# Sanoojan/REFace

Measured on AMD Instinct MI355X. Metric: 512x512 50-step DDIM images/sec, higher is better.
Workload: dtype bf16; 1 GPU; BASELINE configs[1]: 512x512, 50 DDIM steps, CFG scale 3.5, batch 8 per GPU, bf16 UNet + fp32 VAE decode (bf16x3 MFMA operands), seeded random-init REFace weights; id=c1:512x512:S50:B8:bf16, batch_per_gpu=8, global_batch=8, ddim_steps=50, latent=64, parallelism=dp1 (pairs sharded, no collective in the step loop)

## Files before the change

reface_amd/csrc/gemm.hip:

```cpp
#include <cstdlib>
#include <type_traits>

#include "common.h"
#include "gemm_plan.h"


namespace rf {
typedef float f32x2_t __attribute__((ext_vector_type(2)));


typedef __attribute__((ext_vector_type(2))) __bf16 bf16x2v_t;
__device__ __forceinline__ u32x4_t fp8x8_to_bf16x8(const u32x2_t& r, float scale) {
    u32x4_t o;
    o[0] = __builtin_bit_cast(uint32_t, __builtin_amdgcn_cvt_scalef32_pk_bf16_fp8(r[0], scale, false));
    o[1] = __builtin_bit_cast(uint32_t, __builtin_amdgcn_cvt_scalef32_pk_bf16_fp8(r[0], scale, true));
    o[2] = __builtin_bit_cast(uint32_t, __builtin_amdgcn_cvt_scalef32_pk_bf16_fp8(r[1], scale, false));
    o[3] = __builtin_bit_cast(uint32_t, __builtin_amdgcn_cvt_scalef32_pk_bf16_fp8(r[1], scale, true));
    return o;
}

template <typename T> struct MmaFrag;
template <> struct MmaFrag<bf16_t> {
    __device__ static __forceinline__ void mma(f32x16_t& acc, const u32x4_t& a, const u32x4_t& b) {
        acc = __builtin_amdgcn_mfma_f32_32x32x16_bf16(__builtin_bit_cast(bf16x8_t, a), __builtin_bit_cast(bf16x8_t, b), acc, 0, 0, 0);
// ... 27 lines not shown

__device__ __forceinline__ int lds_off(int row, int slot) { return row * 128 + ((slot ^ ((row >> 1) & 7)) << 4); }

template <bool W8> __device__ __forceinline__ int w_stage(int t, int buf) { return W8 ? ((t >> 1) & 1) : buf; }
template <bool W8> __device__ __forceinline__ int w_soff(int t) { return (W8 ? (t >> 1) : t) * 128; }

template <typename TO> __device__ __forceinline__ void store_out(TO* p, float v);
template <> __device__ __forceinline__ void store_out<float>(float* p, float v) { *p = v; }
template <> __device__ __forceinline__ void store_out<bf16_t>(bf16_t* p, float v) { *p = f2bf(v); }
template <> __device__ __forceinline__ void store_out<f16_t>(f16_t* p, float v) { *p = (f16_t)v; }
template <typename TO> __device__ __forceinline__ float load_out(const TO* p);
template <> __device__ __forceinline__ float load_out<float>(const float* p) { return *p; }
template <> __device__ __forceinline__ float load_out<bf16_t>(const bf16_t* p) { return bf2f(*p); }
template <> __device__ __forceinline__ float load_out<f16_t>(const f16_t* p) { return (float)*p; }
template <typename X> struct is16 { static constexpr bool value = std::is_same<X, bf16_t>::value || std::is_same<X, f16_t>::value; };

template <typename T, typename TO, int WM, int WN, int TM, int TN, bool CONV, bool GLDS, int NST, int EPI = 0, bool W8 = false, int LNF = 0, bool HX = false>
__global__ __launch_bounds__(WM* WN * 64) void conv_gemm_kernel(const GemmParams p) {
    static_assert(LNF == 0 || (EPI == 1 && !CONV && !W8 && sizeof(T) == 2 && sizeof(TO) == 2), "LayerNorm folding: bf16 linear layers on the direct epilogue");
    static_assert(!HX || (CONV && GLDS && NST == 2 && sizeof(T) == 2 && !W8), "row-extended A tiles: bf16 3x3 convolutions on the two-stage direct-to-LDS loop");
    static_assert(EPI == 0 || GLDS, "the direct epilogue is built on the direct-to-LDS main loop");
    static_assert(!W8 || (GLDS && std::is_same<T, bf16_t>::value), "fp8 weights: bf16 activations on the direct-to-LDS main loop");
    constexpr bool A8 = std::is_same<T, fp8_t>::value;
    static_assert(!A8 || (GLDS && !W8 && NST == 2), "fp8 activations: direct-to-LDS main loop, two stages");
    constexpr int NT = WM * WN * 64;
    constexpr int BM = 32 * TM * WM;
    constexpr int BN = 32 * TN * WN;
    constexpr int VEC = elem<T>::VEC;
    constexpr int BK = 8 * VEC;
    constexpr int RPP = NT / 8;
// ... 25 lines not shown
        const int h = min(p.pm, p.tiles_m - sr * p.pm);
        const int pw = h * p.pn;
        const int pc = rem / pw, r2 = rem - pc * pw;
        const int c = r2 / h;
        tile_m = sr * p.pm + (r2 - c * h);
        tile_n = pc * p.pn + c;
    }
    const int m0 = tile_m * BM, n0 = tile_n * BN;

    const long long zb = blockIdx.y;
    const T* src0 = (const T*)p.src0 + zb * p.sA;
    const T* src1 = (const T*)p.src1;
    const T* Wp = W8 ? (const T*)((const char*)p.W + zb * p.sW) : (const T*)p.W + zb * p.sW;
    if (!W8 && p.w_ps) Wp += (long long)(m0 / p.rows_per_sample) * p.w_ps;
    const int hw_in = p.Hin * p.Win;
    const int uph = (CONV && p.ups == 2) ? (m0 / hw_in) & 3 : 0;
    if (!W8 && uph) Wp += (long long)uph * p.N * p.ldw;
    const bool up2 = CONV && p.ups == 2;
    const int pad_t = up2 ? 1 - (uph >> 1) : p.pad_t, pad_l = up2 ? 1 - (uph & 1) : p.pad_l;
    auto out_row = [&](int row) -> int {
        if (!up2) return row;
        const int s4 = m0 / (4 * hw_in), r = row - (s4 * 4 + uph) * hw_in;
        const int i = r / p.Win, j = r - i * p.Win;
        return (s4 * p.Hout + 2 * i + (uph >> 1)) * p.Wout + 2 * j + (uph & 1);
    };

    float colc = 0.f;
    if constexpr (EPI == 1) {
        if (tid < BN && n0 + tid < p.N && p.splitk == 1) {
            if (p.bias) colc = p.bias[n0 + tid];
            if (p.rowvec) colc += p.rowvec[(long long)(m0 / p.rows_per_sample) * p.ldv + n0 + tid];
        }
    }
    float colu = 0.f;
    if constexpr (LNF == 2) {
        if (tid < BN && n0 + tid < p.N) colu = p.ln_u[n0 + tid];
    }
    const int r0 = tid >> 3;
    const int slot = GLDS ? ((tid & 7) ^ ((r0 >> 1) & 7)) : (tid & 7);

// ... 159 lines not shown
#pragma unroll
            for (int j = 0; j < BV; ++j)
                __builtin_amdgcn_raw_ptr_buffer_load_lds(rsB, (__attribute__((address_space(3))) void*)(b0 + j * (RPP * 128)), 16, offs[AV + j], so0, 0, 0);
        }
#pragma unroll
        for (int i = 0; i < AV; ++i) {
            const int m = m0 + r0 + i * RPP;
            if constexpr (HX) {
                const int j = r0 + i * RPP, we = p.Wout + 2;
                const int ir = j / we, xc = j - ir * we;
                const int R = m0 / p.Wout + ir;
                const int b = R / p.Hout, oy = R - b * p.Hout;
                rowd[i] = (ir < BM / p.Wout && R * p.Wout < p.M) ? ((unsigned)b << 20 | (unsigned)oy << 10 | (unsigned)xc) : ~0u;
            } else if (CONV) {
                const int hw = p.Hout * p.Wout;
                const int b = m / hw;
                int rem = m - b * hw, wd = p.Wout;
                if (up2) { rem -= uph * hw_in; wd = p.Win; }
                const int oy = rem / wd, ox = rem - oy * wd;
                rowd[i] = m < p.M ? ((unsigned)b << 20 | (unsigned)oy << 10 | (unsigned)ox) : ~0u;
            } else {
                offs[i] = m < p.M ? m * p.ld0 * (int)sizeof(T) + lane_k : OOB;
            }
        }
        auto set_grp = [&](int dy, int ld) {
#pragma unroll
            for (int i = 0; i < AV; ++i) {
                const unsigned d = rowd[i];
                const int iy = (int)((d >> 10) & 1023u) + dy - 1, ix = (int)(d & 1023u) - 1;
                const bool ok = d != ~0u && (unsigned)iy < (unsigned)p.Hin && (unsigned)ix < (unsigned)p.Win;
                offs[i] = ok ? (((int)(d >> 20) * p.Hin + iy) * p.Win + ix) * ld * (int)sizeof(T) + lane_k : OOB;
            }
        };
// ... 618 lines not shown
                        gx[16 + k] = q;
                    }
                }
                if (gn_on) {
                    halfwave_reduce_scatter32(gx, lrow);
                    gcs[((lrow >> 4) * WM + wm) * BN + (wn * TN + j) * 32 + lhalf * 16 + (lrow & 15)] = gx[0];
                }
            }
            if (gn_on) {
                lds_barrier();
                if (tid < 64) {
                    const int c = tid >> 5, g = tid & 31;
                    if (p.gn_part[c]) {
                        const int cpg = p.gn_cpg[c], base = p.gn_coff[c] + n0;
                        const int lo = max(0, g * cpg - base), hi = min(min(BN, p.N - n0), (g + 1) * cpg - base);
                        double sa = 0.0, sq = 0.0;
                        for (int k = lo; k < hi; ++k)
#pragma unroll
                            for (int r = 0; r < WM; ++r) { sa += (double)gcs[r * BN + k]; sq += (double)gcs[(WM + r) * BN + k]; }
                        const int b = m0 / p.gn_rows, mt = (m0 - b * p.gn_rows) / BM;
                        double* o = p.gn_part[c] + (((long long)b * p.gn_nch[c] + p.gn_slot[c] + mt * p.tiles_n + tile_n) * 32 + g) * 2;
                        o[0] = sa;
                        o[1] = sq;
                    }
                }
            }
            if constexpr (ln_p) {
                const int part = (n0 + wn * TN * 32) / (TN * 32);
#pragma unroll
                for (int i = 0; i < TM; ++i) {
                    float sm = 0.f;
#pragma unroll
                    for (int j = 0; j < TN; ++j)
#pragma unroll
                        for (int e = 0; e < 16; ++e) sm += acc[i][j][e];
                    {
                        const auto sw = __builtin_amdgcn_permlane32_swap(as_u32(sm), as_u32(sm), false, false);
                        sm = as_f32(sw[0]) + as_f32(sw[1]);
// ... 123 lines not shown
        float cadd[4] = {0.f, 0.f, 0.f, 0.f};
        const bool rv_uniform = p.rowvec && (p.rows_per_sample % ER == 0);
        if (t_on) {
            const float* rvu = rv_uniform ? p.rowvec + (long long)(mch / p.rows_per_sample) * p.ldv : nullptr;
            if (full) {
                if (p.bias) { const f32x4_t b4 = *(const f32x4_t*)(p.bias + col); cadd[0] = b4[0]; cadd[1] = b4[1]; cadd[2] = b4[2]; cadd[3] = b4[3]; }
                if (rvu) { const f32x4_t r4 = *(const f32x4_t*)(rvu + col); cadd[0] += r4[0]; cadd[1] += r4[1]; cadd[2] += r4[2]; cadd[3] += r4[3]; }
            } else {
#pragma unroll
                for (int e = 0; e < 4; ++e)
                    if (col + e < p.N) { if (p.bias) cadd[e] = p.bias[col + e]; if (rvu) cadd[e] += rvu[col + e]; }
            }
        }
        typedef typename std::conditional<sizeof(TO) == 2, u32x2_t, f32x4_t>::type resv_t;
        int orow_cur = 0, oj = 0, ostep = 0, ostep_j = 0;
        if (up2) {
            const int r = (mch + er) % hw_in, ostep_i = EROWS / p.Win;
            orow_cur = out_row(mch + er);
            oj = r % p.Win;
            ostep_j = EROWS - ostep_i * p.Win;
            ostep = 2 * ostep_i * p.Wout + 2 * ostep_j;
        }
#pragma unroll 1
        for (int k0 = 0; k0 < PASSES; k0 += U) {
            resv_t rq[U];
            bool ok[U];
#pragma unroll
            for (int u = 0; u < U; ++u) {
                const int rl = er + (k0 + u) * EROWS, row = mch + rl;
                ok[u] = t_on && (k0 + u) < PASSES && rl < ER && row < p.M;
                if (ok[u] && resp && full) rq[u] = *(const resv_t*)(resp + (long long)row * p.ldr + col);
            }
#pragma unroll
            for (int u = 0; u < U; ++u) {
                const int orow_u = orow_cur;
                if (up2) {
                    orow_cur += ostep; oj += ostep_j;
                    if (oj >= p.Win) { oj -= p.Win; orow_cur += p.Wout; }
                }
                if (!ok[u]) continue;
                const int rl = er + (k0 + u) * EROWS, row = mch + rl;
                const f32x4_t a4 = *(const f32x4_t*)(stage + rl * BN + cl);
                float v[4] = {a4[0] * p.alpha + cadd[0], a4[1] * p.alpha + cadd[1], a4[2] * p.alpha + cadd[2], a4[3] * p.alpha + cadd[3]};
                if (p.rowvec && !rv_uniform) {
                    const float* rv = p.rowvec + (long long)(row / p.rows_per_sample) * p.ldv;
#pragma unroll
                    for (int e = 0; e < 4; ++e) if (col + e < p.N) v[e] += rv[col + e];
                }
                if (p.act != RF_ACT_NONE) {
#pragma unroll
                    for (int e = 0; e < 4; ++e) {
                        float y = v[e];
                        if (p.act == RF_ACT_SILU) y = silu_exact(y);
                        else if (p.act == RF_ACT_QUICK_GELU) y = quick_gelu(y);
                        else if (p.act == RF_ACT_GELU) y = gelu_erf(y);
                        else if (p.act == RF_ACT_RELU) y = fmaxf(y, 0.0f);
// ... 59 lines not shown
            for (int e = 0; e < 4; ++e) {
                cs[er * BN + cs_ * 4 + e] = gsum[e];
                cs[(EROWS + er) * BN + cs_ * 4 + e] = gsq[e];
            }
        }
        lds_barrier();
        if (tid < 64) {
            const int c = tid >> 5, g = tid & 31;
            if (p.gn_part[c]) {
                const int cpg = p.gn_cpg[c], base = p.gn_coff[c] + n0;
                const int lo = max(0, g * cpg - base), hi = min(min(BN, p.N - n0), (g + 1) * cpg - base);
                double sa = 0.0, sq = 0.0;
                for (int k = lo; k < hi; ++k)
#pragma unroll
                    for (int r = 0; r < EROWS; ++r) { sa += (double)cs[r * BN + k]; sq += (double)cs[(EROWS + r) * BN + k]; }
                const int b = m0 / p.gn_rows, mt = (m0 - b * p.gn_rows) / BM;
                double* o = p.gn_part[c] + (((long long)b * p.gn_nch[c] + p.gn_slot[c] + mt * p.tiles_n + tile_n) * 32 + g) * 2;
                o[0] = sa;
                o[1] = sq;
            }
        }
    }
}

template <typename TO, int SKR>
__global__ __launch_bounds__(256) void splitk_reduce_kernel(const GemmParams p) {
    const int tid = threadIdx.x;
    const int cl = (tid & 63) * 4, rp = tid >> 6;
    const int n0 = blockIdx.x * SK_COLS, m0 = blockIdx.y * SKR;
    const int col = n0 + cl;
    const bool vec = (p.N & 3) == 0 && p.vec_ok;
// ... 135 lines not shown
    for (int z = 1; z < p.splitk; ++z) {
        src += zstride;
        f32x4_t b[4];
#pragma unroll
        for (int q = 0; q < 4; ++q) b[q] = src[q * 64];
#pragma unroll
        for (int q = 0; q < 4; ++q) a[q] += b[q];
    }
    const bool live = row < p.M && col < p.N;
    const bool gn_on = p.gn_rows > 0;
    constexpr int OV = sizeof(TO) == 2 ? 2 : 4, E = 16 / OV;
    float y[16];
#pragma unroll
    for (int e = 0; e < 16; ++e) y[e] = 0.f;
    if (live) {
        TO* const dst = (TO*)p.out + (long long)row * p.ldo + col;
        const TO* const resp = p.residual ? (const TO*)p.residual + (long long)row * p.ldr + col : nullptr;
        const float* const rv = p.rowvec ? p.rowvec + (long long)(row / p.rows_per_sample) * p.ldv + col : nullptr;
        u32x4_t rq[OV];
        if (resp) {
#pragma unroll
            for (int h = 0; h < OV; ++h) rq[h] = ((const u32x4_t*)resp)[h];
        }
#pragma unroll
        for (int q = 0; q < 4; ++q) {
            f32x4_t c = {0.f, 0.f, 0.f, 0.f};
            if (p.bias) c = ((const f32x4_t*)(p.bias + col))[q];
            if (rv) c += ((const f32x4_t*)rv)[q];
#pragma unroll
            for (int e = 0; e < 4; ++e) y[4 * q + e] = a[q][e] * p.alpha + c[e];
        }
// ... 15 lines not shown
    if (gn_on) {
        __shared__ float gcs[2][32 * TN];
        float gx[32];
#pragma unroll
        for (int k = 0; k < 16; ++k) { gx[k] = y[k]; gx[16 + k] = y[k] * y[k]; }
        halfwave_reduce_scatter32(gx, lrow);
        gcs[lrow >> 4][j * 32 + lhalf * 16 + (lrow & 15)] = gx[0];
        __syncthreads();
        if (tid < 64) {
            const int c = tid >> 5, g = tid & 31;
            if (p.gn_part[c] && row0 < p.M && coln0 < p.N) {
                const int cpg = p.gn_cpg[c], base = p.gn_coff[c] + coln0;
                const int lo = max(0, g * cpg - base), hi = min(min(32 * TN, p.N - coln0), (g + 1) * cpg - base);
                double sa = 0.0, sq = 0.0;
                for (int k = lo; k < hi; ++k) { sa += (double)gcs[0][k]; sq += (double)gcs[1][k]; }
                const int b = row0 / p.gn_rows, mt = (row0 - b * p.gn_rows) / 32;
                const int nstripe = (p.N + 32 * TN - 1) / (32 * TN);
                double* o = p.gn_part[c] + (((long long)b * p.gn_nch[c] + p.gn_slot[c] + mt * nstripe + coln0 / (32 * TN)) * 32 + g) * 2;
                o[0] = sa;
                o[1] = sq;
            }
        }
    }
}

#ifdef RF_KERNEL_ONLY
}
#else
template <typename T, typename TO, int TI, bool W8>
static int launch_cfg(const GemmPart& g, const GemmParams& p, bool conv, int batch, hipStream_t st) {
    constexpr GemmTile TILE = GEMM_TILE[TI];
// ... 195 lines not shown
```

reface_amd/csrc/gemm_plan.h:

```cpp
#pragma once
#include <stdint.h>

#include "../../include/reface_hip.h"
#include "check.h"

namespace rf {

struct GemmParams {
    int M, N, K;
    const void* src0;
    const void* src1;
    int C0, Ctot, ld0, ld1;
    int Hin, Win, Hout, Wout, KH, KW, stride, pad_t, pad_l, ups;
    const void* W;
    int ldw;
    const float* bias;
    const float* rowvec;
    int rows_per_sample, ldv;
    const void* residual;
    int ldr, act;
    const float* act_vec;
    void* out;
    int ldo;
    float alpha;
// ... 205 lines not shown
    RF_CHECK(!hx || (tile_hx_ok(t, e) && conv && p.glds && p.KH == 3 && p.KW == 3 && p.stride == 1 && !p.ups && p.pad_t == 1 && p.pad_l == 1 && p.Hin == p.Hout &&
                     p.Win == p.Wout && p.Wout >= 16 && BM % p.Wout == 0 && (BM / p.Wout) * (p.Wout + 2) <= AXR_ &&
                     !(DEEP_OK && (long long)g.tiles_m * g.tiles_n * g.splitk <= 256)),
             "rf_conv_gemm: korder 2 (row-extended A tiles) needs a bf16 3x3 stride-1 pad-1 convolution, Wout >= 16, whose %d-row tile holds whole image rows (Wout = %d) "
             "and that does not take the 4-stage ring", BM, p.Wout);
    RF_CHECK(!(p.ln_out || p.ln_in) || (tile_ln_ok(t, e) && !conv),
             "rf_conv_gemm: LayerNorm folding needs a bf16 linear layer on a direct-epilogue tile (this launch: %d x %d, conv %d)", BM, BN, (int)conv);
    RF_CHECK(!p.ln_in || !d->residual, "rf_conv_gemm: a LayerNorm consumer takes no residual");
    RF_CHECK(!p.ln_out || (direct && d->act == RF_ACT_NONE && p.N % (32 * TN) == 0 && p.ln_out_parts == p.N / (32 * TN)),
             "rf_conv_gemm: ln_stats_out needs the direct epilogue (no split-K, act NONE) and ln_out_parts = N / %d (got %d; direct %d)", 32 * TN, p.ln_out_parts, (int)direct);
    RF_CHECK(!p.ln_in || (direct && p.ln_u && p.ln_in_parts >= 1 && p.ln_in_cols >= 1 && p.ln_eps > 0.f && BN <= 320),
             "rf_conv_gemm: ln_stats_in needs the direct epilogue (no split-K), ln_u, ln_in_parts / ln_in_cols >= 1 and ln_eps > 0 (direct %d)", (int)direct);
    RF_CHECK(p.ups != 2 || (g.splitk == 1 && (p.Hin * p.Win) % BM == 0),
             "rf_conv_gemm: ups 2 needs Hin * Win = %d to be a multiple of the %d-row tile (a tile inside one phase of one sample) and no split-K (this launch: %d)",
             p.Hin * p.Win, BM, g.splitk);
    const bool deep = DEEP_OK && p.glds && !p.x3 && !hx && (long long)g.tiles_m * g.tiles_n * d->batch * g.splitk <= 256;
    g.stages = deep ? tile_deep_stages(t, e) : 2;
    return 0;
}

static inline int check_launch(const rf_conv_gemm_desc* d, const GemmParams& p, const GemmPart& g) {
    if (p.gn_rows > 0) {
        RF_CHECK(p.gn_rows % g.st_rows == 0 && p.M % p.gn_rows == 0 && d->batch == 1 && d->act != RF_ACT_GEGLU,
                 "rf_conv_gemm: fused GroupNorm statistics need gn_rows %% %d == 0 (%d), batch 1, no GEGLU -- ask rf_conv_gemm_plan", g.st_rows, p.gn_rows);
        const int need = (p.gn_rows / g.st_rows) * ((p.N + g.st_cols - 1) / g.st_cols);
        for (int c = 0; c < 2; ++c)
            RF_CHECK(!p.gn_part[c] || (p.gn_cpg[c] > 0 && p.gn_slot[c] >= 0 && p.gn_slot[c] + need <= p.gn_nch[c]),
                     "rf_conv_gemm: GroupNorm consumer %d: cpg=%d slot=%d needs %d slots of %d", c, p.gn_cpg[c], p.gn_slot[c], need, p.gn_nch[c]);
    }
    RF_CHECK(!p.oscale || g.direct, "rf_conv_gemm: fp8 output needs the direct epilogue (8-wave tile, aligned rows, no split-K)");
// ... 11 lines not shown
        if (nt > 0 && mt128 * nt * pick_splitk(d, p, mt128 * nt, bk) >= 160) return n320 ? TILE_128x320 : TILE_128x256;
    } else if (p.glds && d->batch == 1) {
        bool n320 = !geglu && N % 320 == 0;
        if (n320 && N % 256 == 0 && mt256 * (N / 320) >= 192) {
            const long long t320 = mt256 * (N / 320), t256 = mt256 * (N / 256);
            if (((t256 + 255) / 256) * 256 < ((t320 + 255) / 256) * 320) n320 = false;
        }
        const bool n256 = N % 256 == 0 && !n320;
        const long long nt = n320 ? N / 320 : (n256 ? N / 256 : 0);
        if (nt > 0) {
            if (mt256 * nt >= 192) {
                const double rounds = (double)(mt256 * nt) / 256.0, rfill = rounds / (double)((mt256 * nt + 255) / 256);
                const long long tiles_ = mt256 * nt, full_ = tiles_ / 256, rem_ = tiles_ - full_ * 256;
                const long long tail_nt_ = full_ >= 1 && mt256 > 0 ? nt - full_ * 256 / mt256 : 0;
                if (split_n && !n320 && full_ >= 1 && rem_ * 5 >= 256 && rem_ * 5 <= 3 * 256 && (full_ * 256) % mt256 == 0 && mt128 * tail_nt_ >= 192 && p.gn_rows == 0 &&
                    !p.ln_out && !p.oscale && !p.w_ps && !p.x3 && p.ups != 2 && d->batch == 1 && (d->act == RF_ACT_NONE || d->act == RF_ACT_GEGLU)) {
                    *split_n = (int)(full_ * 256 / mt256) * 256;
                    return TILE_256x256;
                }
                if (n320 && (rfill < 0.6 || (rfill < 0.8 && rounds > 1.0) || (d->residual && p.K <= 320))) return TILE_128x160;
                return n320 ? TILE_256x320 : TILE_256x256;
            }
            const int k_rule = p.xt0 != 0x7fffffff ? p.xt0 * bk : p.K;
            if (n320 && k_rule <= 6000 && mt128 * (N / 160) >= 256) return TILE_128x160;
            if (d->act == RF_ACT_NONE) {
                const long long blocks = mt256 * nt * pick_splitk(d, p, mt256 * nt, bk);
                if (blocks > mt256 * nt && blocks <= 4 * mt256 * nt && blocks >= 192 && blocks <= 256) return n320 ? TILE_256x320 : TILE_256x256;
            }
            if (mt128 * nt * pick_splitk(d, p, mt128 * nt, bk) >= 192) return n320 ? TILE_128x320 : TILE_128x256;
        }
    }
    if (geglu) return TILE_128x128;
    if (N <= 64) return TILE_128x64;
    const int pad128 = ((N + 127) / 128) * 128, pad160 = ((N + 159) / 160) * 160;
    return pad160 < pad128 ? TILE_128x160 : TILE_128x128;
}

static inline int plan_conv_gemm(const rf_conv_gemm_desc* d, GemmParams& p, GemmPlan& pl) {
    pl = GemmPlan{};
    RF_CHECK(d != nullptr, "rf_conv_gemm: null descriptor");
    const bool oq = d->out_dtype == RF_FP8_E4M3;
    const bool x3 = d->dtype == RF_BF16X3;
    const bool h16 = d->dtype == RF_F16;
    RF_CHECK(d->dtype == RF_F32 || d->dtype == RF_BF16 || h16 || x3 || d->dtype == RF_FP8_E4M3, "rf_conv_gemm: bad dtype %d", d->dtype);
    RF_CHECK(!h16 || ((d->out_dtype == RF_F16 || d->out_dtype == RF_F32) && d->w_dtype == 0),
             "rf_conv_gemm: fp16 operands write fp16 or fp32 and take fp16 weights (out_dtype %d, w_dtype %d)", d->out_dtype, d->w_dtype);
    RF_CHECK(d->out_dtype != RF_F16 || h16, "rf_conv_gemm: fp16 output needs fp16 operands (dtype %d)", d->dtype);
// ... 101 lines not shown
        p.a_bytes = (unsigned)(p.glds ? ab : 0);
        p.w_bytes = (unsigned)(p.glds ? wb : 0);
        p.ascale = d->ascale; p.as_ld = d->as_ld;
        p.as_bytes = (unsigned)(a8 ? rows_a * d->as_ld : 0);
        p.x3 = x3 ? 1 : 0;
        p.lo_off = x3 ? d->C0 * 2 : 0;
        p.w_ps = d->w_sample_stride;
        RF_CHECK(d->w_sample_stride == 0 || (!conv && !w8 && !a8 && !x3 && d->batch == 1 && d->rows_per_sample > 0 && p.glds &&
                                             d->w_sample_stride >= (long long)(d->N - 1) * p.ldw + d->K),
                 "rf_conv_gemm: w_sample_stride needs a plain bf16 / fp32 GEMM on the direct-to-LDS loop, batch 1, rows_per_sample > 0 and a stride of at least one W");
        if (x3) {
            RF_CHECK(p.glds && (conv || d->C0 == d->K), "rf_conv_gemm: split-bf16 operands need the direct-to-LDS main loop (K and channel count multiples of 64) and C0 == K for plain GEMMs");
            p.K = 3 * d->K;
        }
    }
    RF_CHECK(d->ups >= 0 && d->ups <= 2, "rf_conv_gemm: bad ups %d (0 none, 1 nearest x2 in the addressing, 2 nearest x2 folded into 2x2 phase weights)", d->ups);
    if (d->ups == 2) {
        RF_CHECK((d->dtype == RF_BF16 || h16) && d->w_dtype == 0, "rf_conv_gemm: ups 2 needs bf16 / fp16 operands and weights (dtype %d, w_dtype %d)", d->dtype, d->w_dtype);
        RF_CHECK(d->KH == 2 && d->KW == 2 && d->stride == 1 && d->pad_t == 1 && d->pad_l == 1,
                 "rf_conv_gemm: ups 2 needs KH = KW = 2, stride 1 and pad_t = pad_l = 1, the padding of phase (0, 0) (got %dx%d, stride %d, pad %d %d)", d->KH, d->KW, d->stride, d->pad_t, d->pad_l);
        RF_CHECK(d->Hout == 2 * d->Hin && d->Wout == 2 * d->Win, "rf_conv_gemm: ups 2 needs Hout x Wout = 2 Hin x 2 Win (%dx%d -> %dx%d)", d->Hin, d->Win, d->Hout, d->Wout);
        RF_CHECK(d->C1 == 0 && d->batch == 1, "rf_conv_gemm: ups 2 needs one source and batch 1 (C1 %d, batch %d)", d->C1, d->batch);
        RF_CHECK(!xt && !d->residual && !d->rowvec && !d->ln_stats_in && !d->ln_stats_out && d->w_sample_stride == 0 && d->act != RF_ACT_GEGLU,
                 "rf_conv_gemm: ups 2 takes no tail source (srcx), residual, rowvec, LayerNorm fold, per-sample weights or GEGLU");
        RF_CHECK(d->korder == 0 || d->korder == 1, "rf_conv_gemm: ups 2 needs korder 0 or 1 (got %d)", d->korder);
        RF_CHECK(p.glds, "rf_conv_gemm: ups 2 needs the direct-to-LDS main loop (C0 = %d a multiple of 64, 31-bit operand extents)", d->C0);
    }
    p.wscale = d->wscale;
    const int so = d->out_dtype == RF_F32 ? 4 : 2;
    GemmTypes e;
    if (w8) e = GemmTypes{2, so, true, false};
    else if (x3) e = GemmTypes{2, 4, false, false};
    else if (h16) e = GemmTypes{2, so, false, false};
    else if (a8) e = GemmTypes{1, 2, false, true};
    else {
        RF_CHECK(d->out_dtype != RF_F16, "rf_conv_gemm: fp16 output needs fp16 operands");
        e = GemmTypes{d->dtype == RF_F32 ? 4 : 2, so, false, false};
    }
    pl.types = e;
    pl.conv = conv;
    int n1 = 0;
// ... 19 lines not shown
```

reface_amd/ops.py:

```python
import ctypes as C
import threading

import torch

from . import _lib
from ._lib import (ACT_ADD_RELU, ACT_GEGLU, ACT_GELU, ACT_NONE, ACT_PRELU, ACT_QUICK_GELU, ACT_RELU, ACT_SIGMOID, ACT_SILU, RF_BF16, RF_BF16X3, RF_F16, RF_F32,
                   RF_FP8_E4M3, AttnInDesc, ConvGemmDesc, FfnDesc, StemDesc)

LOG2E = 1.4426950408889634
LN2 = 0.6931471805599453


def code(dt):
    if dt == torch.float32:
        return RF_F32
    if dt == torch.bfloat16:
        return RF_BF16
    if dt == torch.float16:
        return RF_F16
    raise TypeError(f"unsupported dtype {dt}")


H16 = (torch.bfloat16, torch.float16)

# ... 439 lines not shown
    d = StemDesc()
    d.x, d.ldx, d.B, d.H, d.W, d.C = _p(x), x.stride(2), B, H, W_, Cc
    d.w, d.bias, d.out, d.ldo = _p(W), _p(bias), _p(out), out.stride(2)
    d.dup_off = 0
    if dup is not None:
        assert dup.dtype == out.dtype and dup.shape == out.shape and dup.stride() == out.stride()
        off = dup.data_ptr() - out.data_ptr()
        assert off > 0 and off % 16 == 0
        d.dup_off = off // 2
    d.dtype = code(x.dtype)
    return Launch(lib.rf_conv3x3_stem, (C.byref(d),), (d, x, W, bias, out, dup), name)


def conv2d(x, W, out, bias=None, *, ksize=3, stride=1, pad=(1, 1), ups=0, x2=None, residual=None, rowvec=None,
           act=ACT_NONE, act_vec=None, korder=0, x3=False, tail=None, name="conv2d"):
    if ups == 2:
        assert W.dim() == 3 and W.shape[0] == 4 and W.is_contiguous() and ksize == 3 and stride == 1 and tuple(pad) == (1, 1), (tuple(W.shape), ksize, stride, pad)
        assert x2 is None and residual is None and rowvec is None and tail is None and not x3 and not isinstance(x, Fp8Act)
        B, Hin, Win, C0 = x.shape
        assert x.stride(3) == 1 and tuple(out.shape[:3]) == (B, 2 * Hin, 2 * Win) and out.stride(3) == 1 and W.shape[2] == 4 * C0
        return conv_gemm(x, W, out, M=4 * B * Hin * Win, N=out.shape[3], K=4 * C0, C0=C0, ld0=x.stride(2), Hin=Hin, Win=Win, Hout=2 * Hin, Wout=2 * Win,
                         KH=2, KW=2, stride=1, pad_t=1, pad_l=1, ups=2, bias=bias, rows_per_sample=4 * Hin * Win, act=act, act_vec=act_vec,
                         ldo=out.stride(2), korder=korder, name=name)
    if isinstance(x, Fp8Act):
        B, Hin, Win, C0 = x.q.shape
        ld0 = x.q.stride(2)
    else:
        B, Hin, Win, C0 = x.shape
        ld0 = x.stride(2)
        assert x.stride(3) == 1
    C1 = 0 if x2 is None else x2.shape[3]
    Bo, Hout, Wout, N = out.shape
    assert Bo == B and out.stride(3) == 1
    K = W.shape[1]
    if x3:
        assert x2 is None and C0 % 2 == 0 and K % 3 == 0
        C0, K = C0 // 2, K // 3
# ... 818 lines not shown
```

reface_amd/unet.py:

```python
import math

import os

import torch
import torch.nn as nn

from . import ops
from .gnfuse import ProducerTracker
from .modules import ParamTree, flat_state, weights_version
from .params import UNetConfig, unet_param_specs, unet_plan

F32 = torch.float32
H16 = (torch.bfloat16, torch.float16)


class _Pool:

    def __init__(self, device):
        self.device, self.free, self.bytes = device, {}, 0
        self.on_put = None

    def get(self, shape, dtype):
        n = 1
        for s in shape:
# ... 41 lines not shown
        self.hx_on = os.environ.get("REFACE_HX", "1") == "1"
        self.gn_fold_lin = os.environ.get("REFACE_GN_FOLD", "1") == "1"
        self.tail_fuse = os.environ.get("REFACE_TAIL_FUSE", "1") == "1"
        self.n_tail_fused = 0
        self.po_fold = os.environ.get("REFACE_PO_FOLD", "1") == "1"
        self.n_po_folded = 0
        self.front_fuse = os.environ.get("REFACE_FRONT_FUSE", "1") == "1"
        self.n_front_fused = 0
        self.mid_fuse = os.environ.get("REFACE_MID_FUSE", "1") == "1"
        self.n_mid_fused = 0
        self.out_fuse = os.environ.get("REFACE_OUT_FUSE", "1") == "1"
        self.stem_fuse = os.environ.get("REFACE_STEM_FUSE", "1") == "1"
        self.n_stem_fused = 0
        self.ups_fold = os.environ.get("REFACE_UPS_FOLD", "1") != "0"
        self._ups_folded, self.n_ups_folded = set(), 0
        self.sample_split = os.environ.get("REFACE_SAMPLE_SPLIT", "1") == "1"
        self.n_sample_split = 0
        self.gn_fold_maxc = int(os.environ.get("REFACE_GN_FOLD_MAXC", "640"))
        self.n_gn_folded = 0
        self.n_hx = 0
        self.n_skip_folded = 0
        self.n_ln_folded = 0
        self.n_cu = torch.cuda.get_device_properties(device).multi_processor_count if torch.cuda.is_available() else 256
        self.gn_fused = 0
        self.pool = _Pool(device)
        self._wpack = {}
        self.tracker = ProducerTracker()
        self.pool.on_put = self.tracker.forget
        self.sd = {k: v.detach().to(device=device, dtype=F32) for k, v in sd.items()}
        self.plan = unet_plan(cfg)
# ... 140 lines not shown
        cin = x.shape[3]
        if tail is not None:
            assert self.dt in H16 and not self.w8 and not self.x3 and not isinstance(x, ops.Fp8Act)
            xt, tkey, tbkey = tail
            kw = dict(kw, tail=xt)
            bias = self._packed(bkey, ("+", tbkey), lambda: (self.sd[bkey] + self.sd[tbkey]).contiguous())
            wtail = lambda wp: ops.pack_conv_tail(wp, self.sd[tkey].reshape(out.shape[3], xt.shape[3]))
            tk = ("tail", tkey)
        else:
            bias, wtail, tk = self.f32(bkey), (lambda wp: wp), ()
        if isinstance(x, ops.Fp8Act):
            return ops.conv2d(x, self.gw8(ops.pack_conv_weight(self.sd[wkey], F32), 9, cin), out, self.f32(bkey), name=name, **kw)
        if self.x3 and x.dtype == torch.bfloat16:
            self.n_x3 += 1
            return ops.conv2d(x, ops.pack_x3(ops.pack_conv_weight(self.sd[wkey], F32)), out, self.f32(bkey), x3=True, name=name, **kw)
        if (kw.get("ups", 0) == 1 and self.ups_fold and self.dt in H16 and not self.w8 and tail is None and cin % 64 == 0 and kw.get("rowvec") is None
                and kw.get("residual") is None and (x.shape[1] * x.shape[2]) % 128 == 0):
            made = (wkey, "ups2") not in self._wpack
            cand = ops.conv2d(x, self._packed(wkey, "ups2", lambda: ops.pack_ups_weight(self.sd[wkey], self.dt)), out, bias, name=name, **dict(kw, ups=2))
            try:
                ops.gemm_plan2(cand)
                self._ups_folded.add(wkey)
                self.n_ups_folded = len(self._ups_folded)
                return cand
            except ops._lib.RefaceHipError as e:
                if "ups 2 needs Hin * Win" not in str(e):
                    raise
                del cand
                if made:
                    del self._wpack[(wkey, "ups2")]
        ko = ops.conv_korder(cin, self.dt) if self.korder_on else 0
        if (self.hx_on and self.dt in H16 and not self.w8 and not ko and cin % 64 == 0 and kw.get("stride", 1) == 1 and not kw.get("ups", 0)
                and x.shape[1:3] == out.shape[1:3]):
            cand = ops.conv2d(x, self._packed(wkey, ("hx",) + tk if tk else "hx", lambda: wtail(ops.pack_conv_weight(self.sd[wkey], self.dt, korder=2))), out, bias, korder=2,
                              name=name, **kw)
            try:
                ops.gemm_plan2(cand)
                self.n_hx += 1
                return cand
            except Exception:
                pass
        def pack():
            wp = ops.pack_conv_weight(self.sd[wkey], F32, korder=ko)
            return wtail(wp.to(self.dt) if ko or tk else self.gw(wp, cin))
        l = ops.conv2d(x, self._packed(wkey, ("tap", ko) + tk, pack), out, bias, korder=ko, name=name, **kw)
# ... 9 lines not shown

    def _add_conv3(self, x, wkey, out, bkey, name, rowvec=None, residual=None, tail=None, **kw):
        B, k = x.shape[0], 0
        if (self.sample_split and isinstance(x, torch.Tensor) and not isinstance(out, ops.Fp8Act) and self.dt in H16 and not self.x3 and not self.w8
                and kw.get("stride", 1) == 1):
            HWo, N = out.shape[1] * out.shape[2], out.shape[3]
            tn = (N + 319) // 320
            if HWo % 256 == 0 and B > 1:
                ps = (HWo // 256) * tn
                t = B * ps
                full, rem = divmod(t, self.n_cu)
                if full >= 1 and 0 < rem <= self.n_cu // 4:
                    k = (self.n_cu * full) // ps
                    if not (0 < k < B and k * ps >= 0.9 * self.n_cu * full):
                        k = 0
        if not k:
            return self._add(self._conv3(x, wkey, out, bkey, name, tail=tail, **dict(kw, **({"rowvec": rowvec} if rowvec is not None else {}),
                                                                           **({"residual": residual} if residual is not None else {}))), out)
        self.n_sample_split += 1
        for a, b in ((0, k), (k, B)):
            kws = dict(kw)
            if rowvec is not None:
                kws["rowvec"] = rowvec[a:b]
            if residual is not None:
                kws["residual"] = residual[a:b]
            self._add(self._conv3(x[a:b], wkey, out[a:b], bkey, f"{name}[{a}:{b}]", tail=(None if tail is None else (tail[0][a:b],) + tuple(tail[1:])), **kws), out[a:b])

    def _add(self, launch, out=None):
        self.main.append(launch)
        return self.tracker.record(out, launch)

    def _gn(self, x, key, eps, silu, fp8=False, split=False):
        if split:
# ... 539 lines not shown
```

Baseline: 10.38 images/s.

## Add phase-major row ordering for folded nearest-upsample convs on small spatial sizes

Adds an ups=3 mode for the upsample-folded 2x2 phase-weight convolution in which GEMM rows are ordered phase-major across the whole batch instead of per sample. This lets the fold apply when Hin*Win is not a multiple of the 128-row tile (small-resolution decoder upsamples), as long as batch*Hin*Win is. Those layers then avoid the unfolded 3x3 conv on the upsampled input. Output row remapping, GroupNorm partial-statistics slotting and tile choice are adjusted for the new ordering, with per-row out_row computation in the epilogue adding some integer-division cost.

```diff
diff --git a/reface_amd/csrc/gemm.hip b/reface_amd/csrc/gemm.hip
--- a/reface_amd/csrc/gemm.hip
+++ b/reface_amd/csrc/gemm.hip
@@ -65,6 +65,33 @@
 template <> __device__ __forceinline__ float load_out<bf16_t>(const bf16_t* p) { return bf2f(*p); }
 template <> __device__ __forceinline__ float load_out<f16_t>(const f16_t* p) { return (float)*p; }
 template <typename X> struct is16 { static constexpr bool value = std::is_same<X, bf16_t>::value || std::is_same<X, f16_t>::value; };
+
+__device__ __forceinline__ int ups_out_row(const GemmParams& p, int row) {
+    const int hw = p.Hin * p.Win;
+    int s, ph, r;
+    if (p.ups == 2) {
+        const int q = row / hw;
+        r = row - q * hw; s = q >> 2; ph = q & 3;
+    } else {
+        const int bhw = p.M >> 2;
+        ph = row / bhw;
+        const int rem = row - ph * bhw;
+        s = rem / hw; r = rem - s * hw;
+    }
+    const int i = r / p.Win, j = r - i * p.Win;
+    return (s * p.Hout + 2 * i + (ph >> 1)) * p.Wout + 2 * j + (ph & 1);
+}
+__device__ __forceinline__ void gn_block_of(const GemmParams& p, int row0, int rows, int& b, int& mt) {
+    if (p.ups == 3) {
+        const int hw = p.Hin * p.Win, bhw = p.M >> 2;
+        const int ph = row0 / bhw, rem = row0 - ph * bhw;
+        b = rem / hw;
+        mt = (ph * hw + rem - b * hw) / rows;
+    } else {
+        b = row0 / p.gn_rows;
+        mt = (row0 - b * p.gn_rows) / rows;
+    }
+}
 
 template <typename T, typename TO, int WM, int WN, int TM, int TN, bool CONV, bool GLDS, int NST, int EPI = 0, bool W8 = false, int LNF = 0, bool HX = false>
 __global__ __launch_bounds__(WM* WN * 64) void conv_gemm_kernel(const GemmParams p) {
@@ -120,16 +147,12 @@
     const T* Wp = W8 ? (const T*)((const char*)p.W + zb * p.sW) : (const T*)p.W + zb * p.sW;
     if (!W8 && p.w_ps) Wp += (long long)(m0 / p.rows_per_sample) * p.w_ps;
     const int hw_in = p.Hin * p.Win;
-    const int uph = (CONV && p.ups == 2) ? (m0 / hw_in) & 3 : 0;
+    const int uph = !CONV ? 0 : (p.ups == 2 ? (m0 / hw_in) & 3 : (p.ups == 3 ? m0 / (p.M >> 2) : 0));
     if (!W8 && uph) Wp += (long long)uph * p.N * p.ldw;
-    const bool up2 = CONV && p.ups == 2;
+    const bool up2 = CONV && p.ups >= 2;
+    const bool up3 = CONV && p.ups == 3;
     const int pad_t = up2 ? 1 - (uph >> 1) : p.pad_t, pad_l = up2 ? 1 - (uph & 1) : p.pad_l;
-    auto out_row = [&](int row) -> int {
-        if (!up2) return row;
-        const int s4 = m0 / (4 * hw_in), r = row - (s4 * 4 + uph) * hw_in;
-        const int i = r / p.Win, j = r - i * p.Win;
-        return (s4 * p.Hout + 2 * i + (uph >> 1)) * p.Wout + 2 * j + (uph & 1);
-    };
+    auto out_row = [&](int row) -> int { return up2 ? ups_out_row(p, row) : row; };
 
     float colc = 0.f;
     if constexpr (EPI == 1) {
@@ -319,9 +342,14 @@
                 rowd[i] = (ir < BM / p.Wout && R * p.Wout < p.M) ? ((unsigned)b << 20 | (unsigned)oy << 10 | (unsigned)xc) : ~0u;
             } else if (CONV) {
                 const int hw = p.Hout * p.Wout;
-                const int b = m / hw;
+                int b = m / hw;
                 int rem = m - b * hw, wd = p.Wout;
                 if (up2) { rem -= uph * hw_in; wd = p.Win; }
+                if (up3) {
+                    rem = m - uph * (p.M >> 2);
+                    b = rem / hw_in;
+                    rem -= b * hw_in;
+                }
                 const int oy = rem / wd, ox = rem - oy * wd;
                 rowd[i] = m < p.M ? ((unsigned)b << 20 | (unsigned)oy << 10 | (unsigned)ox) : ~0u;
             } else {
@@ -970,14 +998,26 @@
                     if (p.gn_part[c]) {
                         const int cpg = p.gn_cpg[c], base = p.gn_coff[c] + n0;
                         const int lo = max(0, g * cpg - base), hi = min(min(BN, p.N - n0), (g + 1) * cpg - base);
-                        double sa = 0.0, sq = 0.0;
-                        for (int k = lo; k < hi; ++k)
-#pragma unroll
-                            for (int r = 0; r < WM; ++r) { sa += (double)gcs[r * BN + k]; sq += (double)gcs[(WM + r) * BN + k]; }
-                        const int b = m0 / p.gn_rows, mt = (m0 - b * p.gn_rows) / BM;
-                        double* o = p.gn_part[c] + (((long long)b * p.gn_nch[c] + p.gn_slot[c] + mt * p.tiles_n + tile_n) * 32 + g) * 2;
-                        o[0] = sa;
-                        o[1] = sq;
+                        if (up3) {
+                            for (int r = 0; r < WM; ++r) {
+                                double sa = 0.0, sq = 0.0;
+                                for (int k = lo; k < hi; ++k) { sa += (double)gcs[r * BN + k]; sq += (double)gcs[(WM + r) * BN + k]; }
+                                int b, mt;
+                                gn_block_of(p, m0 + r * (32 * TM), 32 * TM, b, mt);
+                                double* o = p.gn_part[c] + (((long long)b * p.gn_nch[c] + p.gn_slot[c] + mt * p.tiles_n + tile_n) * 32 + g) * 2;
+                                o[0] = sa;
+                                o[1] = sq;
+                            }
+                        } else {
+                            double sa = 0.0, sq = 0.0;
+                            for (int k = lo; k < hi; ++k)
+#pragma unroll
+                                for (int r = 0; r < WM; ++r) { sa += (double)gcs[r * BN + k]; sq += (double)gcs[(WM + r) * BN + k]; }
+                            const int b = m0 / p.gn_rows, mt = (m0 - b * p.gn_rows) / BM;
+                            double* o = p.gn_part[c] + (((long long)b * p.gn_nch[c] + p.gn_slot[c] + mt * p.tiles_n + tile_n) * 32 + g) * 2;
+                            o[0] = sa;
+                            o[1] = sq;
+                        }
                     }
                 }
             }
@@ -1131,7 +1171,7 @@
         }
         typedef typename std::conditional<sizeof(TO) == 2, u32x2_t, f32x4_t>::type resv_t;
         int orow_cur = 0, oj = 0, ostep = 0, ostep_j = 0;
-        if (up2) {
+        if (up2 && !up3) {
             const int r = (mch + er) % hw_in, ostep_i = EROWS / p.Win;
             orow_cur = out_row(mch + er);
             oj = r % p.Win;
@@ -1150,13 +1190,14 @@
             }
 #pragma unroll
             for (int u = 0; u < U; ++u) {
-                const int orow_u = orow_cur;
-                if (up2) {
+                int orow_u = orow_cur;
+                if (up2 && !up3) {
                     orow_cur += ostep; oj += ostep_j;
                     if (oj >= p.Win) { oj -= p.Win; orow_cur += p.Wout; }
                 }
                 if (!ok[u]) continue;
                 const int rl = er + (k0 + u) * EROWS, row = mch + rl;
+                if (up3) orow_u = out_row(row);
                 const f32x4_t a4 = *(const f32x4_t*)(stage + rl * BN + cl);
                 float v[4] = {a4[0] * p.alpha + cadd[0], a4[1] * p.alpha + cadd[1], a4[2] * p.alpha + cadd[2], a4[3] * p.alpha + cadd[3]};
                 if (p.rowvec && !rv_uniform) {
@@ -1246,7 +1287,8 @@
                 for (int k = lo; k < hi; ++k)
 #pragma unroll
                     for (int r = 0; r < EROWS; ++r) { sa += (double)cs[r * BN + k]; sq += (double)cs[(EROWS + r) * BN + k]; }
-                const int b = m0 / p.gn_rows, mt = (m0 - b * p.gn_rows) / BM;
+                int b, mt;
+                gn_block_of(p, m0, BM, b, mt);
                 double* o = p.gn_part[c] + (((long long)b * p.gn_nch[c] + p.gn_slot[c] + mt * p.tiles_n + tile_n) * 32 + g) * 2;
                 o[0] = sa;
                 o[1] = sq;
@@ -1412,7 +1454,7 @@
 #pragma unroll
     for (int e = 0; e < 16; ++e) y[e] = 0.f;
     if (live) {
-        TO* const dst = (TO*)p.out + (long long)row * p.ldo + col;
+        TO* const dst = (TO*)p.out + (long long)(p.ups >= 2 ? ups_out_row(p, row) : row) * p.ldo + col;
         const TO* const resp = p.residual ? (const TO*)p.residual + (long long)row * p.ldr + col : nullptr;
         const float* const rv = p.rowvec ? p.rowvec + (long long)(row / p.rows_per_sample) * p.ldv + col : nullptr;
         u32x4_t rq[OV];
@@ -1458,7 +1500,8 @@
                 const int lo = max(0, g * cpg - base), hi = min(min(32 * TN, p.N - coln0), (g + 1) * cpg - base);
                 double sa = 0.0, sq = 0.0;
                 for (int k = lo; k < hi; ++k) { sa += (double)gcs[0][k]; sq += (double)gcs[1][k]; }
-                const int b = row0 / p.gn_rows, mt = (row0 - b * p.gn_rows) / 32;
+                int b, mt;
+                gn_block_of(p, row0, 32, b, mt);
                 const int nstripe = (p.N + 32 * TN - 1) / (32 * TN);
                 double* o = p.gn_part[c] + (((long long)b * p.gn_nch[c] + p.gn_slot[c] + mt * nstripe + coln0 / (32 * TN)) * 32 + g) * 2;
                 o[0] = sa;
diff --git a/reface_amd/csrc/gemm_plan.h b/reface_amd/csrc/gemm_plan.h
--- a/reface_amd/csrc/gemm_plan.h
+++ b/reface_amd/csrc/gemm_plan.h
@@ -243,6 +243,18 @@
     RF_CHECK(p.ups != 2 || (g.splitk == 1 && (p.Hin * p.Win) % BM == 0),
              "rf_conv_gemm: ups 2 needs Hin * Win = %d to be a multiple of the %d-row tile (a tile inside one phase of one sample) and no split-K (this launch: %d)",
              p.Hin * p.Win, BM, g.splitk);
+    if (p.ups == 3) {
+        const int hw = p.Hin * p.Win;
+        RF_CHECK((p.M / 4) % BM == 0 && hw % 32 == 0,
+                 "rf_conv_gemm: ups 3 needs B * Hin * Win = %d to be a multiple of the %d-row tile (a tile inside one phase) and Hin * Win = %d a multiple of 32 (a 32-row block inside one sample)",
+                 p.M / 4, BM, hw);
+        RF_CHECK(g.splitk == 1 || g.frag,
+                 "rf_conv_gemm: ups 3 needs the fragment-slab reduce pass for split-K (this launch: %d): a direct-epilogue tile (this launch: %d x %d), 16-byte aligned rows, workspace for the slabs",
+                 g.splitk, BM, BN);
+        if (g.splitk == 1 && direct) g.st_rows = 32 * TM;
+        RF_CHECK(hw % g.st_rows == 0, "rf_conv_gemm: ups 3 needs Hin * Win = %d to be a multiple of the %d rows of a statistics slot (this launch: %d x %d tile, direct epilogue %d)",
+                 hw, g.st_rows, BM, BN, (int)direct);
+    }
     const bool deep = DEEP_OK && p.glds && !p.x3 && !hx && (long long)g.tiles_m * g.tiles_n * d->batch * g.splitk <= 256;
     g.stages = deep ? tile_deep_stages(t, e) : 2;
     return 0;
@@ -284,7 +296,7 @@
                 const long long tiles_ = mt256 * nt, full_ = tiles_ / 256, rem_ = tiles_ - full_ * 256;
                 const long long tail_nt_ = full_ >= 1 && mt256 > 0 ? nt - full_ * 256 / mt256 : 0;
                 if (split_n && !n320 && full_ >= 1 && rem_ * 5 >= 256 && rem_ * 5 <= 3 * 256 && (full_ * 256) % mt256 == 0 && mt128 * tail_nt_ >= 192 && p.gn_rows == 0 &&
-                    !p.ln_out && !p.oscale && !p.w_ps && !p.x3 && p.ups != 2 && d->batch == 1 && (d->act == RF_ACT_NONE || d->act == RF_ACT_GEGLU)) {
+                    !p.ln_out && !p.oscale && !p.w_ps && !p.x3 && p.ups < 2 && d->batch == 1 && (d->act == RF_ACT_NONE || d->act == RF_ACT_GEGLU)) {
                     *split_n = (int)(full_ * 256 / mt256) * 256;
                     return TILE_256x256;
                 }
@@ -301,6 +313,7 @@
         }
     }
     if (geglu) return TILE_128x128;
+    if (p.ups == 3 && (p.Hin * p.Win) % 128 != 0) return TILE_128x160;
     if (N <= 64) return TILE_128x64;
     const int pad128 = ((N + 127) / 128) * 128, pad160 = ((N + 159) / 160) * 160;
     return pad160 < pad128 ? TILE_128x160 : TILE_128x128;
@@ -432,17 +445,21 @@
             p.K = 3 * d->K;
         }
     }
-    RF_CHECK(d->ups >= 0 && d->ups <= 2, "rf_conv_gemm: bad ups %d (0 none, 1 nearest x2 in the addressing, 2 nearest x2 folded into 2x2 phase weights)", d->ups);
-    if (d->ups == 2) {
-        RF_CHECK((d->dtype == RF_BF16 || h16) && d->w_dtype == 0, "rf_conv_gemm: ups 2 needs bf16 / fp16 operands and weights (dtype %d, w_dtype %d)", d->dtype, d->w_dtype);
+    RF_CHECK(d->ups >= 0 && d->ups <= 3,
+             "rf_conv_gemm: bad ups %d (0 none, 1 nearest x2 in the addressing, 2 nearest x2 folded into 2x2 phase weights, 3 the same with phase-major rows)", d->ups);
+    if (d->ups >= 2) {
+        const int u = d->ups;
+        RF_CHECK((d->dtype == RF_BF16 || h16) && d->w_dtype == 0, "rf_conv_gemm: ups %d needs bf16 / fp16 operands and weights (dtype %d, w_dtype %d)", u, d->dtype, d->w_dtype);
         RF_CHECK(d->KH == 2 && d->KW == 2 && d->stride == 1 && d->pad_t == 1 && d->pad_l == 1,
-                 "rf_conv_gemm: ups 2 needs KH = KW = 2, stride 1 and pad_t = pad_l = 1, the padding of phase (0, 0) (got %dx%d, stride %d, pad %d %d)", d->KH, d->KW, d->stride, d->pad_t, d->pad_l);
-        RF_CHECK(d->Hout == 2 * d->Hin && d->Wout == 2 * d->Win, "rf_conv_gemm: ups 2 needs Hout x Wout = 2 Hin x 2 Win (%dx%d -> %dx%d)", d->Hin, d->Win, d->Hout, d->Wout);
-        RF_CHECK(d->C1 == 0 && d->batch == 1, "rf_conv_gemm: ups 2 needs one source and batch 1 (C1 %d, batch %d)", d->C1, d->batch);
+                 "rf_conv_gemm: ups %d needs KH = KW = 2, stride 1 and pad_t = pad_l = 1, the padding of phase (0, 0) (got %dx%d, stride %d, pad %d %d)", u, d->KH, d->KW, d->stride, d->pad_t, d->pad_l);
+        RF_CHECK(d->Hout == 2 * d->Hin && d->Wout == 2 * d->Win, "rf_conv_gemm: ups %d needs Hout x Wout = 2 Hin x 2 Win (%dx%d -> %dx%d)", u, d->Hin, d->Win, d->Hout, d->Wout);
+        RF_CHECK(d->C1 == 0 && d->batch == 1, "rf_conv_gemm: ups %d needs one source and batch 1 (C1 %d, batch %d)", u, d->C1, d->batch);
         RF_CHECK(!xt && !d->residual && !d->rowvec && !d->ln_stats_in && !d->ln_stats_out && d->w_sample_stride == 0 && d->act != RF_ACT_GEGLU,
-                 "rf_conv_gemm: ups 2 takes no tail source (srcx), residual, rowvec, LayerNorm fold, per-sample weights or GEGLU");
-        RF_CHECK(d->korder == 0 || d->korder == 1, "rf_conv_gemm: ups 2 needs korder 0 or 1 (got %d)", d->korder);
-        RF_CHECK(p.glds, "rf_conv_gemm: ups 2 needs the direct-to-LDS main loop (C0 = %d a multiple of 64, 31-bit operand extents)", d->C0);
+                 "rf_conv_gemm: ups %d takes no tail source (srcx), residual, rowvec, LayerNorm fold, per-sample weights or GEGLU", u);
+        RF_CHECK(u != 3 || d->rows_per_sample == d->Hin * d->Win,
+                 "rf_conv_gemm: ups 3: rows_per_sample must be Hin * Win = %d, a sample's run of consecutive rows inside a phase (got %d)", d->Hin * d->Win, d->rows_per_sample);
+        RF_CHECK(d->korder == 0 || d->korder == 1, "rf_conv_gemm: ups %d needs korder 0 or 1 (got %d)", u, d->korder);
+        RF_CHECK(p.glds, "rf_conv_gemm: ups %d needs the direct-to-LDS main loop (C0 = %d a multiple of 64, 31-bit operand extents)", u, d->C0);
     }
     p.wscale = d->wscale;
     const int so = d->out_dtype == RF_F32 ? 4 : 2;
diff --git a/reface_amd/ops.py b/reface_amd/ops.py
--- a/reface_amd/ops.py
+++ b/reface_amd/ops.py
@@ -477,13 +477,13 @@
 
 def conv2d(x, W, out, bias=None, *, ksize=3, stride=1, pad=(1, 1), ups=0, x2=None, residual=None, rowvec=None,
            act=ACT_NONE, act_vec=None, korder=0, x3=False, tail=None, name="conv2d"):
-    if ups == 2:
+    if ups in (2, 3):
         assert W.dim() == 3 and W.shape[0] == 4 and W.is_contiguous() and ksize == 3 and stride == 1 and tuple(pad) == (1, 1), (tuple(W.shape), ksize, stride, pad)
         assert x2 is None and residual is None and rowvec is None and tail is None and not x3 and not isinstance(x, Fp8Act)
         B, Hin, Win, C0 = x.shape
         assert x.stride(3) == 1 and tuple(out.shape[:3]) == (B, 2 * Hin, 2 * Win) and out.stride(3) == 1 and W.shape[2] == 4 * C0
         return conv_gemm(x, W, out, M=4 * B * Hin * Win, N=out.shape[3], K=4 * C0, C0=C0, ld0=x.stride(2), Hin=Hin, Win=Win, Hout=2 * Hin, Wout=2 * Win,
-                         KH=2, KW=2, stride=1, pad_t=1, pad_l=1, ups=2, bias=bias, rows_per_sample=4 * Hin * Win, act=act, act_vec=act_vec,
+                         KH=2, KW=2, stride=1, pad_t=1, pad_l=1, ups=ups, bias=bias, rows_per_sample=(4 if ups == 2 else 1) * Hin * Win, act=act, act_vec=act_vec,
                          ldo=out.stride(2), korder=korder, name=name)
     if isinstance(x, Fp8Act):
         B, Hin, Win, C0 = x.q.shape
diff --git a/reface_amd/unet.py b/reface_amd/unet.py
--- a/reface_amd/unet.py
+++ b/reface_amd/unet.py
@@ -79,6 +79,8 @@
         self.n_stem_fused = 0
         self.ups_fold = os.environ.get("REFACE_UPS_FOLD", "1") != "0"
         self._ups_folded, self.n_ups_folded = set(), 0
+        self._ups_phase_major, self.n_ups_phase_major = set(), 0
+        self.ups_pm_min_rows = int(os.environ.get("REFACE_UPS_PM_MIN_ROWS", "2048"))
         self.sample_split = os.environ.get("REFACE_SAMPLE_SPLIT", "1") == "1"
         self.n_sample_split = 0
         self.gn_fold_maxc = int(os.environ.get("REFACE_GN_FOLD_MAXC", "640"))
@@ -249,21 +251,27 @@
         if self.x3 and x.dtype == torch.bfloat16:
             self.n_x3 += 1
             return ops.conv2d(x, ops.pack_x3(ops.pack_conv_weight(self.sd[wkey], F32)), out, self.f32(bkey), x3=True, name=name, **kw)
+        hw_in = x.shape[1] * x.shape[2]
         if (kw.get("ups", 0) == 1 and self.ups_fold and self.dt in H16 and not self.w8 and tail is None and cin % 64 == 0 and kw.get("rowvec") is None
-                and kw.get("residual") is None and (x.shape[1] * x.shape[2]) % 128 == 0):
+                and kw.get("residual") is None and (x.shape[0] * hw_in) % 128 == 0 and hw_in % 32 == 0):
             made = (wkey, "ups2") not in self._wpack
-            cand = ops.conv2d(x, self._packed(wkey, "ups2", lambda: ops.pack_ups_weight(self.sd[wkey], self.dt)), out, bias, name=name, **dict(kw, ups=2))
-            try:
-                ops.gemm_plan2(cand)
-                self._ups_folded.add(wkey)
-                self.n_ups_folded = len(self._ups_folded)
-                return cand
-            except ops._lib.RefaceHipError as e:
-                if "ups 2 needs Hin * Win" not in str(e):
-                    raise
-                del cand
-                if made:
-                    del self._wpack[(wkey, "ups2")]
+            wf = self._packed(wkey, "ups2", lambda: ops.pack_ups_weight(self.sd[wkey], self.dt))
+            for u, refusal, seen in ((2, "ups 2 needs Hin * Win", self._ups_folded), (3, "ups 3 needs", self._ups_phase_major)):
+                if (u == 2 and hw_in % 128) or (u == 3 and x.shape[0] * hw_in < self.ups_pm_min_rows):
+                    continue
+                cand = ops.conv2d(x, wf, out, bias, name=name, **dict(kw, ups=u))
+                try:
+                    ops.gemm_plan2(cand)
+                    seen.add(wkey)
+                    self.n_ups_folded, self.n_ups_phase_major = len(self._ups_folded), len(self._ups_phase_major)
+                    return cand
+                except ops._lib.RefaceHipError as e:
+                    if refusal not in str(e):
+                        raise
+                    del cand
+            del wf
+            if made:
+                del self._wpack[(wkey, "ups2")]
         ko = ops.conv_korder(cin, self.dt) if self.korder_on else 0
         if (self.hx_on and self.dt in H16 and not self.w8 and not ko and cin % 64 == 0 and kw.get("stride", 1) == 1 and not kw.get("ups", 0)
                 and x.shape[1:3] == out.shape[1:3]):
@@ -303,9 +311,15 @@
                     k = (self.n_cu * full) // ps
                     if not (0 < k < B and k * ps >= 0.9 * self.n_cu * full):
                         k = 0
+        whole = lambda: self._conv3(x, wkey, out, bkey, name, tail=tail, **dict(kw, **({"rowvec": rowvec} if rowvec is not None else {}),
+                                                                                **({"residual": residual} if residual is not None else {})))
+        if k and kw.get("ups", 0) == 1 and self.ups_fold and (x.shape[1] * x.shape[2]) % 128:
+            l = whole()
+            if l.keep[0].ups == 3:
+                return self._add(l, out)
+            del l
         if not k:
-            return self._add(self._conv3(x, wkey, out, bkey, name, tail=tail, **dict(kw, **({"rowvec": rowvec} if rowvec is not None else {}),
-                                                                           **({"residual": residual} if residual is not None else {}))), out)
+            return self._add(whole(), out)
         self.n_sample_split += 1
         for a, b in ((0, k), (k, B)):
             kws = dict(kw)
```

Result: no change. 10.37 images/s (-0.0%).
